# jcbowden/EagleEverything

Measured on NVIDIA B200. Metric: markers/s, higher is better.
Workload: dtype f64

## Files before the change

### eagleeverything_b200/csrc/capi.cu

```cuda
#include <cublas_v2.h>
#include <dlfcn.h>
#include <fcntl.h>
#include <sys/mman.h>
#include <sys/stat.h>
#include <unistd.h>

#include <cmath>
#include <cstdarg>
#include <cstdlib>
#include <cstring>
#include <atomic>
#include <condition_variable>
#include <functional>
#include <mutex>
#include <thread>
#include <unordered_map>
#include <string>
#include <vector>

#include "common.cuh"
#include "hostio.cuh"

struct eg_store {
    int8_t* d = nullptr;
// ... 74 lines not shown
    int dev = 0, sms = 0;
    if (cudaGetDevice(&dev) == cudaSuccess &&
        cudaDeviceGetAttribute(&sms, cudaDevAttrMultiProcessorCount, dev) == cudaSuccess && sms > 0)
        return sms;
    return 148;
}

static int ensure_init() {
    if (g_ctx.ready) return check_cuda(cudaSetDevice(g_ctx.device), "cudaSetDevice");
    const char* env = getenv("EAGLE_GPU_DEVICE");
    return eg_init(env ? atoi(env) : 0);
}

int ensure_init_pub() { return ensure_init(); }
cudaStream_t ctx_stream() { return g_ctx.stream; }
cublasHandle_t ctx_cublas() { return g_ctx.cublas; }

void syrk_release_cache();
void scan_i8_release();
void algebra_release();
void eigbasis_release();
void prep_i8_release();
int launch_prepare_i8(const double* d_S, const double* d_V, int64_t n, int64_t col0, int64_t col1, double* d_tmp,
                      double* d_Wp, int64_t Kpad, cudaStream_t st, bool* done);
static int g_scan_mode = -1;
int scan_mode() {
    if (g_scan_mode < 0) {
        const char* e = getenv("EAGLE_SCAN_MODE");
        g_scan_mode = (e && (e[0] == 'f' || e[0] == 'd' || e[0] == '0')) ? 0 : 1;
    }
    return g_scan_mode;
}
int launch_scan(const int8_t* d_Mt, int64_t L, int64_t n, int64_t pitch, const double* d_Wp,
                const int64_t* d_zero_rows, int n_zero, double* d_a, double* d_vara, cudaStream_t st);

#define g_pool_mu g_ctx.pool_mu
#define g_free_blocks g_ctx.free_blocks
#define g_live_blocks g_ctx.live_blocks
#define g_free_bytes g_ctx.free_bytes
#define g_recycle_limit g_ctx.recycle_limit

static void pool_flush_locked() {
    for (auto& b : g_free_blocks) cudaFreeAsync(b.p, g_ctx.stream);
    g_free_blocks.clear();
    g_free_bytes = 0;
}
static cudaError_t pool_alloc(void** p, size_t bytes) {
// ... 425 lines not shown
    cache_insert(key, s);
    *out = s;
    return EG_OK;
}

__global__ void __launch_bounds__(256) i8_to_f64_colmajor_kernel(const int8_t* __restrict__ in, int64_t rows,
                                                                 int64_t cols, int64_t pitch,
                                                                 double* __restrict__ out) {
    __shared__ int8_t tile[32][33];
    const int tx = threadIdx.x & 31, ty = threadIdx.x >> 5;
    const int64_t r0 = (int64_t)blockIdx.y * 32, c0 = (int64_t)blockIdx.x * 32;
    for (int i = ty; i < 32; i += 8) {
        const int64_t r = r0 + i, c = c0 + tx;
        tile[i][tx] = (r < rows && c < cols) ? in[r * pitch + c] : (int8_t)0;
    }
    __syncthreads();
    for (int i = ty; i < 32; i += 8) {
        const int64_t c = c0 + i, r = r0 + tx;
        if (r < rows && c < cols) out[r + c * rows] = -(double)tile[tx][i];
    }
}

__global__ void __launch_bounds__(256) symmetrize_upper_kernel(double* __restrict__ Wp, int64_t n, int64_t ld,
                                                               int w_is_upper) {
    __shared__ double tile[32][33];
    const int bx = blockIdx.x, by = blockIdx.y;
    if (bx < by) return;
    const int tx = threadIdx.x & 31, ty = threadIdx.x >> 5;
    const int64_t r0 = (int64_t)by * 32, c0 = (int64_t)bx * 32;
    for (int i = ty; i < 32; i += 8) {
        const int64_t r = c0 + tx, c = r0 + i;
        tile[i][tx] = (r < n && c < n) ? Wp[r + c * ld] : 0.0;
    }
    __syncthreads();
    for (int i = ty; i < 32; i += 8) {
        const int64_t r = r0 + tx, c = c0 + i;
        if (r < n && c < n) {
            if (r < c) Wp[r + c * ld] = Wp[r + c * ld] + (w_is_upper ? Wp[r + c * ld] : tile[tx][i]);
            else if (r > c) Wp[r + c * ld] = 0.0;
        }
    }
    if (bx != by) {
        __syncthreads();
        for (int i = ty; i < 32; i += 8) {
            const int64_t r = c0 + tx, c = r0 + i;
            if (r < n && c < n) Wp[r + c * ld] = 0.0;
        }
// ... 23 lines not shown
        const int64_t r = r0 + tx, c = c0 + i;
        v[k] = (r < n && c < n) ? A[r + c * n] : 0.0;
    }
    double mabs = 0.0, masym = 0.0;
#pragma unroll
    for (int k = 0; k < 16; k++) {
        const int i = ty + 4 * k;
        if (r0 + tx < n && c0 + i < n) {
            const double a = v[k], b = tile[tx][i];
            mabs = fmax(mabs, fmax(fabs(a), fabs(b)));
            const double d = fabs(a - b);
            masym = fmax(masym, d == d ? d : 1.0e300);
        }
    }
#pragma unroll
    for (int o = 16; o > 0; o >>= 1) {
        mabs = fmax(mabs, __shfl_xor_sync(0xffffffffu, mabs, o));
        masym = fmax(masym, __shfl_xor_sync(0xffffffffu, masym, o));
    }
    if ((threadIdx.x & 31) == 0) {
        atomicMax(out, (unsigned long long)__double_as_longlong(mabs));
        atomicMax(out + 1, (unsigned long long)__double_as_longlong(masym));
    }
}

static int partial_product(const eg_store* M, const std::vector<int64_t>& zero_cols, DevBuf& C, bool keep_product);
static int mmt_of_composite(const eg_store* M, const std::vector<int64_t>& zero_cols, double* out_host, bool keep_product);
static int scan_of_composite(const eg_store* Mt, const std::vector<int64_t>& zero_rows, const double* S, const double* V,
                             const double* a, double* out_a, double* out_vara);
static int mmt_of_store(const eg_store* M, const std::vector<int64_t>& zero_cols, double* out_host, bool keep_product = false) {
    Pin pin(M);
    if (M->nparts > 1) return mmt_of_composite(M, zero_cols, out_host, keep_product);
    const int64_t n = M->rows;
    DevBuf C, D;
    EG_TRY(partial_product(M, zero_cols, C, keep_product));
    EG_TRY(D.alloc((size_t)n * n * sizeof(double), "MMt output"));
    cudaStream_t st = g_ctx.stream;
    {
        Timer t(st);
        EG_TRY(eg_dev_mmt_finalize(C.as<int32_t>(), n, n, D.as<double>(), st));
        g_ctx.timing[2] = t.stop();
    }
    {
        Timer t(st);
        EG_TRY(d2h_staged(out_host, D.p, (size_t)n * n * sizeof(double), st));
        g_ctx.timing[3] = t.stop();
// ... 913 lines not shown
    const int64_t Kpad = round_up(n, 32), nc = col1 - col0;
    const bool want_i8 = eg_prep_uses_i8(n) != 0;
    if (upper_only && want_i8) {
        bool done = false;
        EG_TRY(launch_prepare_i8(d_S, d_V, n, col0, col1, d_tmp, d_Wp, Kpad, st, &done));
        if (done) return EG_OK;
    }
    const double one = 1.0, zero = 0.0;
    if (cublasSetStream(g_ctx.cublas, st) != CUBLAS_STATUS_SUCCESS) return set_error(EG_ERR_CUDA, "cublasSetStream");
    if (cublasDgemm(g_ctx.cublas, CUBLAS_OP_N, CUBLAS_OP_N, (int)n, (int)nc, (int)n, &one, d_V, (int)n, d_S + col0 * n,
                    (int)n, &zero, d_tmp, (int)n) != CUBLAS_STATUS_SUCCESS)
        return set_error(EG_ERR_CUDA, "cublasDgemm(V*S) failed");
    const int64_t step = upper_only ? 1024 : nc;
    for (int64_t b0 = 0; b0 < nc; b0 += step) {
        const int64_t nb = (b0 + step <= nc) ? step : nc - b0;
        const int64_t rows = upper_only ? (col0 + b0 + nb) : n;
        if (cublasDgemm(g_ctx.cublas, CUBLAS_OP_N, CUBLAS_OP_N, (int)rows, (int)nb, (int)n, &one, d_S, (int)n,
                        d_tmp + b0 * n, (int)n, &zero, d_Wp + (col0 + b0) * Kpad, (int)Kpad) != CUBLAS_STATUS_SUCCESS)
            return set_error(EG_ERR_CUDA, "cublasDgemm(S*tmp) failed");
    }
    return EG_OK;
}

extern "C" int eg_dev_scan_fold(const double* d_S, const double* d_a, int64_t n, int w_is_upper, double* d_Wp,
                                void* stream) {
    if (!d_S || !d_a || !d_Wp || n <= 0) return set_error(EG_ERR_ARG, "eg_dev_scan_fold: bad argument");
    EG_TRY(ensure_init());
    cudaStream_t st = (cudaStream_t)stream;
    const int64_t Kpad = round_up(n, 32);
    const double one = 1.0, zero = 0.0;
    if (cublasSetStream(g_ctx.cublas, st) != CUBLAS_STATUS_SUCCESS) return set_error(EG_ERR_CUDA, "cublasSetStream");
    if (cublasDgemv(g_ctx.cublas, CUBLAS_OP_N, (int)n, (int)n, &one, d_S, (int)n, d_a, 1, &zero, d_Wp + n * Kpad, 1) !=
        CUBLAS_STATUS_SUCCESS)
        return set_error(EG_ERR_CUDA, "cublasDgemv(S*a) failed");
    const unsigned nb = (unsigned)((n + 31) / 32);
    symmetrize_upper_kernel<<<dim3(nb, nb), 256, 0, st>>>(d_Wp, n, Kpad, w_is_upper);
    return check_launch("symmetrize_upper_kernel");
}

extern "C" int eg_dev_inputs_symmetric(const double* d_S, const double* d_V, int64_t n, int* yes, void* stream) {
    if (!yes) return set_error(EG_ERR_ARG, "null");
    double aS, dS, aV, dV;
    EG_TRY(eg_dev_symmetry(d_S, n, &aS, &dS, stream));
    EG_TRY(eg_dev_symmetry(d_V, n, &aV, &dV, stream));
    const char* env = getenv("EAGLE_SCAN_SYMMETRIC");
    *yes = !(env && env[0] == '0') && dS <= 1e-13 * aS && dV <= 1e-13 * aV;
    return EG_OK;
}

extern "C" int eg_dev_scan_prepare(const double* d_S, const double* d_V, const double* d_a, int64_t n, double* d_tmp,
                                   double* d_Wp, void* stream) {
    if (!d_S || !d_V || !d_a || !d_tmp || !d_Wp || n <= 0) return set_error(EG_ERR_ARG, "eg_dev_scan_prepare: bad argument");
    EG_TRY(ensure_init());
    int sym = 0;
    EG_TRY(eg_dev_inputs_symmetric(d_S, d_V, n, &sym, stream));
    EG_CUDA(cudaMemsetAsync(d_Wp, 0, (size_t)eg_scan_wp_elems(n) * 8, (cudaStream_t)stream));
    EG_TRY(eg_dev_scan_prepare_cols(d_S, d_V, n, 0, n, sym, d_tmp, d_Wp, stream));
    return eg_dev_scan_fold(d_S, d_a, n, sym, d_Wp, stream);
}

extern "C" int eg_ReadBlock(const char* asciifname, int64_t start_row, int64_t numcols, int64_t numrows_in_block,
                            double* out_colmajor) {
    if (!asciifname || !out_colmajor || start_row < 0 || numcols <= 0 || numrows_in_block <= 0)
        return set_error(EG_ERR_ARG, "ReadBlock: bad argument");
    EG_TRY(ensure_init());
    MappedFile f;
    EG_TRY(f.open_ro(asciifname));
    const void* nl = memchr(f.p, '\n', f.size);
    const int64_t line = nl ? (const uint8_t*)nl - f.p : (int64_t)f.size;
    if (numcols > line) return set_error(EG_ERR_FORMAT, "ReadBlock: lines of %s have %lld characters, %lld requested",
                                         asciifname, (long long)line, (long long)numcols);
    const int64_t nrows_file = ((int64_t)f.size + 1) / (line + 1);
    if (start_row + numrows_in_block > nrows_file)
        return set_error(EG_ERR_FORMAT, "ReadBlock: %s has %lld lines, rows [%lld,%lld) requested", asciifname,
                         (long long)nrows_file, (long long)start_row, (long long)(start_row + numrows_in_block));
    eg_store* s = nullptr;
// ... 651 lines not shown
```

### eagleeverything_b200/csrc/prep_i8.cu

```cuda
#include <cstdlib>
#include <vector>

#include "common.cuh"
#include "ptx.cuh"

namespace eg {

constexpr int PI_BM = 128;
constexpr int PI_BN = 256;
constexpr int PI_BK = 128;
constexpr int PI_STAGES = 4;
constexpr int PI_A_BYTES = PI_BM * PI_BK;
constexpr int PI_B_BYTES = PI_BN * PI_BK;
constexpr int PI_STAGE_BYTES = PI_A_BYTES + PI_B_BYTES;
constexpr int PI_THREADS = 192;
constexpr int PI_TMEM_COLS = 512;
constexpr int PI_SLICES = 7;
constexpr int PI_LEVELS = 7;
constexpr int PI_TERMS = PI_LEVELS * (PI_LEVELS + 1) / 2;
constexpr int PI_SMEM_BYTES = PI_STAGES * PI_STAGE_BYTES + 1024 + 256;
constexpr int PI_SROWS = 12;
constexpr int PI_PHASE = 8;
constexpr int PI_LAG = 4;

struct PrepParams {
    int64_t M, N, ld;
    double* out;
    const double* sL;
    const double* sR;
    int32_t lrow0, rrow0;
    int32_t KB;
    int64_t diag_shift;
    int32_t upper_only;
    const int2* tiles;
    int32_t ntiles, nchunks, ngroups;
    uint8_t tp[PI_TERMS], tq[PI_TERMS];
    uint8_t cbeg[PI_TERMS + 1];
    double cw[PI_TERMS];
    uint32_t* phase_ctr;
    int32_t phases_per_tile, phase_len, lag;
};

__device__ __forceinline__ void pi_red_add(uint32_t* p, uint32_t v) {
    asm volatile("red.relaxed.gpu.global.add.u32 [%0], %1;" ::"l"(p), "r"(v) : "memory");
}
__device__ __forceinline__ uint32_t pi_ld(const uint32_t* p) {
    uint32_t v;
    asm volatile("ld.relaxed.gpu.global.u32 %0, [%1];" : "=r"(v) : "l"(p) : "memory");
    return v;
}

__global__ void __launch_bounds__(PI_THREADS, 1)
prep_i8_kernel(const __grid_constant__ CUtensorMap tmapL, const __grid_constant__ CUtensorMap tmapR, const PrepParams p) {
    extern __shared__ uint8_t smem_raw[];
    uint8_t* smem = reinterpret_cast<uint8_t*>((reinterpret_cast<uintptr_t>(smem_raw) + 1023) & ~(uintptr_t)1023);
    uint64_t* bars = reinterpret_cast<uint64_t*>(smem + PI_STAGES * PI_STAGE_BYTES);
    uint64_t* full = bars;
    uint64_t* empty = bars + PI_STAGES;
    uint64_t* tmem_full = bars + 2 * PI_STAGES;
    uint64_t* tmem_empty = tmem_full + 2;
    uint32_t* tmem_slot = reinterpret_cast<uint32_t*>(tmem_empty + 2);

    const int warp = threadIdx.x >> 5, lane = threadIdx.x & 31;
    if (warp == 0 && lane == 0) {
        ptx::prefetch_tmap(&tmapL);
        ptx::prefetch_tmap(&tmapR);
        for (int s = 0; s < PI_STAGES; s++) {
            ptx::mbar_init(&full[s], 1);
            ptx::mbar_init(&empty[s], 1);
        }
        for (int a = 0; a < 2; a++) {
            ptx::mbar_init(&tmem_full[a], 1);
            ptx::mbar_init(&tmem_empty[a], 4);
        }
        ptx::fence_mbar_init();
    }
    if (warp == 1) ptx::tmem_alloc<PI_TMEM_COLS>(tmem_slot);
    ptx::tc_fence_before();
    __syncthreads();
    ptx::tc_fence_after();
    const uint32_t tmem_base = *tmem_slot;

    const int nun = p.ngroups * p.nchunks;

    if (warp == 0) {
// ... 85 lines not shown
                if (++acc == 2) { acc = 0; acc_phase ^= 1; }
            }
        }
    } else {
        const int q = warp & 3;
        int acc = 0;
        uint32_t acc_phase = 0;
        for (int u = 0; u < nun; u++) {
            const int gi = u / p.nchunks, c = u - gi * p.nchunks;
            const int tile = gi * (int)gridDim.x + (int)blockIdx.x;
            if (tile >= p.ntiles) break;
            const int2 t = p.tiles[tile];
            const bool first = c == 0, last = c == p.nchunks - 1;
            const double w = p.cw[c];
            const int64_t row0 = (int64_t)t.x * PI_BM + q * 32;
            const int64_t row = row0 + lane;
            const double srow = (last && row < p.M) ? p.sL[row] * 281474976710656.0  : 0.0;
            ptx::mbar_wait(&tmem_full[acc], acc_phase);
            ptx::tc_fence_after();
#pragma unroll 1
            for (int cc = 0; cc < PI_BN / 32; cc++) {
                const int64_t col0 = (int64_t)t.y * PI_BN + cc * 32;
                if (col0 >= p.N) continue;
                if (p.upper_only && col0 + 31 + p.diag_shift < row0) continue;
                uint32_t v[32];
                ptx::tmem_ld_32x32(tmem_base + ((uint32_t)(q * 32) << 16) + (uint32_t)(acc * PI_BN + cc * 32), v);
                double* o = p.out + row + col0 * p.ld;
                const bool live = row < p.M;
                double run[32];
#pragma unroll
                for (int j = 0; j < 32; j++) run[j] = (live && !first && col0 + j < p.N) ? o[(int64_t)j * p.ld] : 0.0;
                ptx::tmem_ld_wait();
                if (live) {
#pragma unroll
                    for (int j = 0; j < 32; j++) {
                        if (col0 + j < p.N) {
                            double x = w * (double)(int)v[j];
                            if (!first) x += run[j];
                            if (last) x *= srow * __ldg(p.sR + col0 + j);
                            o[(int64_t)j * p.ld] = x;
                        }
                    }
                }
            }
            ptx::tc_fence_before();
            __syncwarp();
            if (lane == 0) ptx::mbar_arrive(&tmem_empty[acc]);
// ... 6 lines not shown
    if (warp == 1) {
        ptx::tc_fence_after();
        ptx::tmem_dealloc<PI_TMEM_COLS>(tmem_base);
    }
}

constexpr int PP_STAGES = 6;
constexpr int PP_B_BYTES = 128 * PI_BK;
constexpr int PP_STAGE_BYTES = PI_A_BYTES + PP_B_BYTES;
constexpr int PP_SMEM_BYTES = PP_STAGES * PP_STAGE_BYTES + 1024 + 256;
constexpr int PP_BM = 2 * PI_BM;

__global__ void __launch_bounds__(PI_THREADS, 1)
prep_i8_pair_kernel(const __grid_constant__ CUtensorMap tmapL, const __grid_constant__ CUtensorMap tmapR, const PrepParams p) {
    extern __shared__ uint8_t smem_raw[];
    uint8_t* smem = reinterpret_cast<uint8_t*>((reinterpret_cast<uintptr_t>(smem_raw) + 1023) & ~(uintptr_t)1023);
    uint64_t* bars = reinterpret_cast<uint64_t*>(smem + PP_STAGES * PP_STAGE_BYTES);
    uint64_t* full = bars;
    uint64_t* empty = bars + PP_STAGES;
    uint64_t* tmem_full = bars + 2 * PP_STAGES;
    uint64_t* tmem_empty = tmem_full + 2;
    uint32_t* tmem_slot = reinterpret_cast<uint32_t*>(tmem_empty + 2);

    const int warp = threadIdx.x >> 5, lane = threadIdx.x & 31;
    const uint32_t rank = ptx::cluster_ctarank();
    const int cid = (int)ptx::cluster_id_x();
    const int ncl = (int)gridDim.x / 2;
    if (warp == 0 && lane == 0) {
        ptx::prefetch_tmap(&tmapL);
        ptx::prefetch_tmap(&tmapR);
        for (int s = 0; s < PP_STAGES; s++) {
            ptx::mbar_init(&full[s], 1);
            ptx::mbar_init(&empty[s], 1);
        }
        for (int a = 0; a < 2; a++) {
            ptx::mbar_init(&tmem_full[a], 1);
            ptx::mbar_init(&tmem_empty[a], 8);
        }
        ptx::fence_mbar_init();
    }
    if (warp == 1) ptx::tmem_alloc_pair<PI_TMEM_COLS>(tmem_slot);
    ptx::tc_fence_before();
    ptx::cluster_sync();
    ptx::tc_fence_after();
    const uint32_t tmem_base = *tmem_slot;

// ... 88 lines not shown
                if (++acc == 2) { acc = 0; acc_phase ^= 1; }
            }
        }
    } else {
        const int q = warp & 3;
        int acc = 0;
        uint32_t acc_phase = 0;
        for (int u = 0; u < nun; u++) {
            const int gi = u / p.nchunks, c = u - gi * p.nchunks;
            const int tile = gi * ncl + cid;
            if (tile >= p.ntiles) break;
            const int2 t = p.tiles[tile];
            const bool first = c == 0, last = c == p.nchunks - 1;
            const double w = p.cw[c];
            const int64_t row0 = (int64_t)t.x * PP_BM + (int64_t)rank * PI_BM + q * 32;
            const int64_t row = row0 + lane;
            const double srow = (last && row < p.M) ? p.sL[row] * 281474976710656.0  : 0.0;
            ptx::mbar_wait(&tmem_full[acc], acc_phase);
            ptx::tc_fence_after();
#pragma unroll 1
            for (int cc = 0; cc < PI_BN / 32; cc++) {
                const int64_t col0 = (int64_t)t.y * PI_BN + cc * 32;
                if (col0 >= p.N) continue;
                if (p.upper_only && col0 + 31 + p.diag_shift < row0) continue;
                uint32_t v[32];
                ptx::tmem_ld_32x32(tmem_base + ((uint32_t)(q * 32) << 16) + (uint32_t)(acc * PI_BN + cc * 32), v);
                double* o = p.out + row + col0 * p.ld;
                const bool live = row < p.M;
                double run[32];
#pragma unroll
                for (int j = 0; j < 32; j++) run[j] = (live && !first && col0 + j < p.N) ? o[(int64_t)j * p.ld] : 0.0;
                ptx::tmem_ld_wait();
                if (live) {
#pragma unroll
                    for (int j = 0; j < 32; j++) {
                        if (col0 + j < p.N) {
                            double x = w * (double)(int)v[j];
                            if (!first) x += run[j];
                            if (last) x *= srow * __ldg(p.sR + col0 + j);
                            o[(int64_t)j * p.ld] = x;
                        }
                    }
                }
            }
            ptx::tc_fence_before();
            __syncwarp();
            if (lane == 0) ptx::mbar_arrive_cluster(ptx::mapa(ptx::smem_u32(&tmem_empty[acc]), 0));
            if (++acc == 2) { acc = 0; acc_phase ^= 1; }
        }
    }

    ptx::tc_fence_before();
    ptx::cluster_sync();
    if (warp == 1) {
        ptx::tc_fence_after();
        ptx::tmem_dealloc_pair<PI_TMEM_COLS>(tmem_base);
    }
}

__global__ void __launch_bounds__(256) pi_colscale_kernel(const double* __restrict__ A, int64_t rows, int64_t ld,
                                                          int32_t* __restrict__ expo, double* __restrict__ scale,
                                                          const double* __restrict__ rowscale) {
    const int64_t c = blockIdx.x;
    unsigned long long m = 0;
    for (int64_t i = threadIdx.x; i < rows; i += 256) {
        const double x = rowscale ? A[i + c * ld] * rowscale[i] : A[i + c * ld];
        const unsigned long long b = (unsigned long long)__double_as_longlong(x) & 0x7FFFFFFFFFFFFFFFull;
        m = b > m ? b : m;
    }
    __shared__ unsigned long long sh[8];
#pragma unroll
    for (int o = 16; o > 0; o >>= 1) {
        const unsigned long long other = __shfl_xor_sync(0xffffffffu, m, o);
        m = other > m ? other : m;
    }
    if ((threadIdx.x & 31) == 0) sh[threadIdx.x >> 5] = m;
    __syncthreads();
    if (threadIdx.x == 0) {
        for (int w = 1; w < 8; w++) m = sh[w] > m ? sh[w] : m;
        const double amax = __longlong_as_double((long long)m);
        int e = 0;
        double s = 0.0;
        if (m >= 0x7FF0000000000000ull) {
            s = __longlong_as_double(0x7FF8000000000000LL);
        } else if (amax > 0.0) {
            if (frexp(amax, &e) >= 0.9921875) e++;
            s = ldexp(1.0, e - 55);
        }
        expo[c] = e;
        scale[c] = s;
    }
}
__global__ void __launch_bounds__(256) pi_slice_kernel(const double* __restrict__ A, int64_t rows, int64_t ld,
                                                       const int32_t* __restrict__ expo, int8_t* __restrict__ Q, int64_t Kp,
                                                       int64_t slice_stride, const double* __restrict__ rowscale) {
    const int64_t c = blockIdx.y;
    const int64_t i0 = ((int64_t)blockIdx.x * 256 + threadIdx.x) * 4;
    if (i0 >= Kp) return;
    uint32_t out[PI_SLICES];
#pragma unroll
    for (int s = 0; s < PI_SLICES; s++) out[s] = 0;
    const int e = expo[c];
#pragma unroll
    for (int d = 0; d < 4; d++) {
        const int64_t i = i0 + d;
        if (i < rows) {
            const double xs = ldexp(rowscale ? A[i + c * ld] * rowscale[i] : A[i + c * ld], 55 - e);
            long long X = fabs(xs) < 3.6e16 ? __double2ll_rn(xs) : 0;
#pragma unroll
            for (int s = PI_SLICES - 1; s > 0; s--) {
                const int q = (int)(int8_t)(X & 0xFF);
                out[s] |= ((uint32_t)q & 0xFFu) << (8 * d);
                X = (X - q) >> 8;
            }
            out[0] |= ((uint32_t)(int)X & 0xFFu) << (8 * d);
        }
    }
    int8_t* base = Q + c * Kp + i0;
#pragma unroll
    for (int s = 0; s < PI_SLICES; s++) *reinterpret_cast<uint32_t*>(base + (int64_t)s * slice_stride) = out[s];
}

typedef CUresult (*PFN_encodeTiled)(CUtensorMap*, CUtensorMapDataType, cuuint32_t, void*, const cuuint64_t*,
                                    const cuuint64_t*, const cuuint32_t*, const cuuint32_t*, CUtensorMapInterleave,
                                    CUtensorMapSwizzle, CUtensorMapL2promotion, CUtensorMapFloatOOBfill);
static PFN_encodeTiled pi_encode_fn() {
    static PFN_encodeTiled fn = nullptr;
    if (!fn) {
        void* f = nullptr;
        cudaDriverEntryPointQueryResult qres;
        if (cudaGetDriverEntryPoint("cuTensorMapEncodeTiled", &f, cudaEnableDefault, &qres) == cudaSuccess &&
            qres == cudaDriverEntryPointSuccess)
            fn = reinterpret_cast<PFN_encodeTiled>(f);
    }
    return fn;
}
static int pi_make_map(CUtensorMap* m, const void* base, int64_t Kp, int64_t rows) {
    PFN_encodeTiled enc = pi_encode_fn();
    if (!enc) return set_error(EG_ERR_CUDA, "cuTensorMapEncodeTiled is not available");
    const cuuint64_t gdim[3] = {(cuuint64_t)Kp, (cuuint64_t)rows, (cuuint64_t)PI_SLICES};
    const cuuint64_t gstride[2] = {(cuuint64_t)Kp, (cuuint64_t)(Kp * rows)};
    const cuuint32_t box[3] = {128, 128, 1};
    const cuuint32_t estr[3] = {1, 1, 1};
    CUresult r = enc(m, CU_TENSOR_MAP_DATA_TYPE_UINT8, 3, const_cast<void*>(base), gdim, gstride, box, estr,
                     CU_TENSOR_MAP_INTERLEAVE_NONE, CU_TENSOR_MAP_SWIZZLE_128B, CU_TENSOR_MAP_L2_PROMOTION_L2_256B,
                     CU_TENSOR_MAP_FLOAT_OOB_FILL_NONE);
    if (r != CUDA_SUCCESS) return set_error(EG_ERR_CUDA, "cuTensorMapEncodeTiled failed (%d)", (int)r);
    return EG_OK;
}

static bool prep_i8_pair() {
    const char* e = getenv("EAGLE_PREP_PAIR");
    return e && e[0] == '1';
}

struct PrepWorkspace {
    int device = -1;
    int8_t* qS = nullptr;  size_t qS_cap = 0;
    int8_t* qV = nullptr;  size_t qV_cap = 0;
    int8_t* qX = nullptr;  size_t qX_cap = 0;
    double* sc = nullptr;  size_t sc_cap = 0;
    int32_t* ex = nullptr; size_t ex_cap = 0;
    int2* tiles = nullptr; size_t tiles_cap = 0;
    uint32_t* phase = nullptr; size_t phase_cap = 0;
};
static thread_local PrepWorkspace g_pi;

static thread_local cudaEvent_t g_pi_ev[4] = {nullptr, nullptr, nullptr, nullptr};
static thread_local double g_pi_ops = 0.0;
static thread_local int g_pi_marks = 0;
void prep_kernel_times(double* ms, double* ops) {
    *ms = 0.0;
    *ops = g_pi_ops;
    for (int i = 0; i + 1 < g_pi_marks; i += 2) {
        float f = 0.f;
        if (cudaEventSynchronize(g_pi_ev[i + 1]) == cudaSuccess && cudaEventElapsedTime(&f, g_pi_ev[i], g_pi_ev[i + 1]) == cudaSuccess)
            *ms += f;
    }
}

void prep_i8_release() {
    cudaFree(g_pi.qS); cudaFree(g_pi.qV); cudaFree(g_pi.qX); cudaFree(g_pi.sc); cudaFree(g_pi.ex); cudaFree(g_pi.tiles); cudaFree(g_pi.phase);
    g_pi = PrepWorkspace();
}
template <class T>
static bool pi_grow(T** ptr, size_t* cap, size_t need) {
    if (need <= *cap && *ptr) return true;
    if (*ptr) cudaFree(*ptr);
    *ptr = nullptr;
    *cap = 0;
    if (malloc_retry((void**)ptr, need * sizeof(T)) != cudaSuccess) {
        cudaGetLastError();
        return false;
    }
    *cap = need;
    return true;
}

static int pi_slice(const double* d_A, int64_t rows, int64_t ld, int64_t ncols, int8_t* Q, int64_t Kp, int32_t* expo,
                    double* scale, cudaStream_t st, const double* d_rowscale = nullptr) {
    pi_colscale_kernel<<<(unsigned)ncols, 256, 0, st>>>(d_A, rows, ld, expo, scale, d_rowscale);
    EG_TRY(check_launch("pi_colscale_kernel"));
    pi_slice_kernel<<<dim3((unsigned)((Kp / 4 + 255) / 256), (unsigned)ncols), 256, 0, st>>>(d_A, rows, ld, expo, Q, Kp,
                                                                                          Kp * ncols, d_rowscale);
    return check_launch("pi_slice_kernel");
}

static int pi_product(const int8_t* qL, int64_t lrows, const double* sL, int64_t lrow0, int64_t M, const int8_t* qR,
                      int64_t rrows, const double* sR, int64_t rrow0, int64_t N, int64_t n, int64_t Kp, double* out,
                      int64_t ld, bool upper_only, int64_t diag_shift, cudaStream_t st) {
    const bool pair = prep_i8_pair();
    const int BMt = pair ? PP_BM : PI_BM;
    const int TM = (int)((M + BMt - 1) / BMt), TN = (int)((N + PI_BN - 1) / PI_BN);
    std::vector<int2> h;
    int srows = PI_SROWS;
    if (const char* e = getenv("EAGLE_PREP_SROWS")) srows = atoi(e) > 0 ? atoi(e) : srows;
    if (pair) srows = (srows + 1) / 2;
    for (int sr = 0; sr < TM; sr += srows)
        for (int tj = 0; tj < TN; tj++)
            for (int ti = sr; ti < TM && ti < sr + srows; ti++) {
                if (upper_only && (int64_t)(tj + 1) * PI_BN - 1 + diag_shift < (int64_t)ti * BMt) continue;
                h.push_back(make_int2(ti, tj));
            }
    if (h.empty()) return EG_OK;
    if (!pi_grow(&g_pi.tiles, &g_pi.tiles_cap, h.size())) return set_error(EG_ERR_ALLOC, "prep_i8: tile table");
    EG_CUDA(cudaMemcpyAsync(g_pi.tiles, h.data(), h.size() * sizeof(int2), cudaMemcpyHostToDevice, st));
    EG_CUDA(cudaStreamSynchronize(st));

    PrepParams p;
    p.M = M; p.N = N; p.ld = ld; p.out = out;
    p.sL = sL + lrow0; p.sR = sR + rrow0;
    p.lrow0 = (int32_t)lrow0; p.rrow0 = (int32_t)rrow0;
    p.KB = (int32_t)(Kp / PI_BK);
    p.diag_shift = diag_shift;
    p.upper_only = upper_only ? 1 : 0;
    p.tiles = g_pi.tiles;
    p.ntiles = (int32_t)h.size();
    const int64_t tmax64 = (((int64_t)1 << 31) - 1) / (n * 16384);
    const int tmax = (int)(tmax64 > PI_LEVELS ? PI_LEVELS : tmax64);
    if (tmax < 1) return set_error(EG_ERR_ARG, "prep_i8: n = %lld too large for int32 accumulation", (long long)n);
    int nt = 0, nc = 0;
    for (int d = PI_LEVELS - 1; d >= 0; d--) {
        for (int p0 = 0; p0 <= d; p0 += tmax) {
            p.cbeg[nc] = (uint8_t)nt;
            double w = 1.0;
            for (int e = 0; e < PI_LEVELS - 1 - d; e++) w *= 256.0;
            p.cw[nc] = w;
            for (int pp = p0; pp <= d && pp < p0 + tmax; pp++) {
                p.tp[nt] = (uint8_t)pp;
                p.tq[nt] = (uint8_t)(d - pp);
                nt++;
            }
            nc++;
        }
    }
    p.cbeg[nc] = (uint8_t)nt;
    p.nchunks = nc;
    const int sms = num_sms();
    const int workers_max = pair ? sms / 2 : sms;
    const int workers = p.ntiles < workers_max ? p.ntiles : workers_max;
    const int grid = pair ? 2 * workers : workers;
    p.ngroups = (p.ntiles + workers - 1) / workers;

    CUtensorMap tL, tR;
    EG_TRY(pi_make_map(&tL, qL, Kp, lrows));
    EG_TRY(pi_make_map(&tR, qR, Kp, rrows));
    if (pair) EG_CUDA(cudaFuncSetAttribute(prep_i8_pair_kernel, cudaFuncAttributeMaxDynamicSharedMemorySize, PP_SMEM_BYTES));
    else EG_CUDA(cudaFuncSetAttribute(prep_i8_kernel, cudaFuncAttributeMaxDynamicSharedMemorySize, PI_SMEM_BYTES));
    p.phase_len = PI_PHASE;
    p.lag = PI_LAG;
    if (const char* e = getenv("EAGLE_PREP_PHASE")) p.phase_len = atoi(e) > 0 ? atoi(e) : p.phase_len;
    if (const char* e = getenv("EAGLE_PREP_LAG")) p.lag = atoi(e) > 0 && atoi(e) <= 8 ? atoi(e) : p.lag;
    p.phases_per_tile = (nt * p.KB + p.phase_len - 1) / p.phase_len;
    const size_t nctr = (size_t)p.ngroups * p.phases_per_tile;
    const char* env_fc = getenv("EAGLE_PREP_FLOWCTL");
    const bool flow = !(env_fc && env_fc[0] == '0') && workers > 1;
    p.phase_ctr = nullptr;
    if (flow) {
        if (!pi_grow(&g_pi.phase, &g_pi.phase_cap, nctr)) return set_error(EG_ERR_ALLOC, "prep_i8: flow-control counters");
        EG_CUDA(cudaMemsetAsync(g_pi.phase, 0, nctr * sizeof(uint32_t), st));
        p.phase_ctr = g_pi.phase;
    }
    cudaLaunchConfig_t cfg = {};
    cfg.gridDim = dim3((unsigned)grid);
    cfg.blockDim = dim3(PI_THREADS);
    cfg.dynamicSmemBytes = pair ? PP_SMEM_BYTES : PI_SMEM_BYTES;
    cfg.stream = st;
    cudaLaunchAttribute attr[2];
    attr[0].id = cudaLaunchAttributeCooperative;
    attr[0].val.cooperative = flow ? 1 : 0;
    attr[1].id = cudaLaunchAttributeClusterDimension;
    attr[1].val.clusterDim.x = 2;
    attr[1].val.clusterDim.y = 1;
    attr[1].val.clusterDim.z = 1;
    cfg.attrs = attr;
    cfg.numAttrs = pair ? 2 : 1;
    if (!g_pi_ev[0])
        for (int i = 0; i < 4; i++) cudaEventCreate(&g_pi_ev[i]);
    if (g_pi_marks <= 2) {
        cudaEventRecord(g_pi_ev[g_pi_marks], st);
        g_pi_ops += (double)p.ntiles * nt * p.KB * 2.0 * BMt * PI_BN * PI_BK;
    }
    if (pair) EG_CUDA(cudaLaunchKernelEx(&cfg, prep_i8_pair_kernel, tL, tR, p));
    else EG_CUDA(cudaLaunchKernelEx(&cfg, prep_i8_kernel, tL, tR, p));
    if (g_pi_marks <= 2) {
        cudaEventRecord(g_pi_ev[g_pi_marks + 1], st);
        g_pi_marks += 2;
    }
    return check_launch("prep_i8_kernel");
}

int launch_prepare_i8(const double* d_S, const double* d_V, int64_t n, int64_t col0, int64_t col1, double* d_tmp,
                      double* d_Wp, int64_t Kpad, cudaStream_t st, bool* done) {
    *done = false;
    g_pi_marks = 0;
    g_pi_ops = 0.0;
    int dev = 0;
    EG_CUDA(cudaGetDevice(&dev));
    if (g_pi.device != dev) {
        if (g_pi.device >= 0) prep_i8_release();
        g_pi.device = dev;
    }
    if (n * 16384 >= ((int64_t)1 << 31)) return EG_OK;
    const int64_t Kp = round_up(n, 128), nc = col1 - col0;
    size_t free_b = 0, total_b = 0;
    EG_CUDA(cudaMemGetInfo(&free_b, &total_b));
    const size_t need = (size_t)PI_SLICES * Kp * (size_t)(2 * n + nc);
    const size_t have = g_pi.qS_cap + g_pi.qV_cap + g_pi.qX_cap;
    if (need > have && need - have + ((size_t)2 << 30) > free_b) return EG_OK;
    if (!pi_grow(&g_pi.qS, &g_pi.qS_cap, (size_t)PI_SLICES * Kp * n) || !pi_grow(&g_pi.qV, &g_pi.qV_cap, (size_t)PI_SLICES * Kp * n) ||
        !pi_grow(&g_pi.qX, &g_pi.qX_cap, (size_t)PI_SLICES * Kp * nc) || !pi_grow(&g_pi.sc, &g_pi.sc_cap, (size_t)(2 * n + nc)) ||
        !pi_grow(&g_pi.ex, &g_pi.ex_cap, (size_t)(2 * n + nc)))
        return EG_OK;
    double *sS = g_pi.sc, *sV = g_pi.sc + n, *sX = g_pi.sc + 2 * n;
    int32_t *eS = g_pi.ex, *eV = g_pi.ex + n, *eX = g_pi.ex + 2 * n;
    EG_TRY(pi_slice(d_S, n, n, n, g_pi.qS, Kp, eS, sS, st));
    EG_TRY(pi_slice(d_V, n, n, n, g_pi.qV, Kp, eV, sV, st));
    EG_TRY(pi_product(g_pi.qV, n, sV, 0, n, g_pi.qS, n, sS, col0, nc, n, Kp, d_tmp, n, false, 0, st));
    EG_TRY(pi_slice(d_tmp, n, n, nc, g_pi.qX, Kp, eX, sX, st));
    EG_TRY(pi_product(g_pi.qS, n, sS, 0, col1, g_pi.qX, nc, sX, 0, nc, n, Kp, d_Wp + col0 * Kpad, Kpad, true, col0, st));
    *done = true;
    return EG_OK;
}

int launch_prepare_eig_i8(const double* d_Ut, const double* d_rs, int64_t n, double* d_Wp, int64_t Kpad, cudaStream_t st,
                          bool* done) {
    *done = false;
    g_pi_marks = 0;
    g_pi_ops = 0.0;
    int dev = 0;
    EG_CUDA(cudaGetDevice(&dev));
    if (g_pi.device != dev) {
        if (g_pi.device >= 0) prep_i8_release();
        g_pi.device = dev;
    }
    if (n * 16384 >= ((int64_t)1 << 31)) return EG_OK;
    const int64_t Kp = round_up(n, 128);
    size_t free_b = 0, total_b = 0;
    EG_CUDA(cudaMemGetInfo(&free_b, &total_b));
    const size_t need = (size_t)PI_SLICES * Kp * (size_t)n;
    if (need > g_pi.qS_cap && need - g_pi.qS_cap + ((size_t)2 << 30) > free_b) return EG_OK;
    if (!pi_grow(&g_pi.qS, &g_pi.qS_cap, need) || !pi_grow(&g_pi.sc, &g_pi.sc_cap, (size_t)n) ||
        !pi_grow(&g_pi.ex, &g_pi.ex_cap, (size_t)n))
        return EG_OK;
    EG_TRY(pi_slice(d_Ut, n, n, n, g_pi.qS, Kp, g_pi.ex, g_pi.sc, st, d_rs));
    EG_TRY(pi_product(g_pi.qS, n, g_pi.sc, 0, n, g_pi.qS, n, g_pi.sc, 0, n, n, Kp, d_Wp, Kpad, true, 0, st));
    *done = true;
    return EG_OK;
}

}
```

Baseline: 2.949 million.

## Decide scan-prepare symmetry on device and cache tile tables to remove host syncs

The symmetry check for S and V now stays on the GPU: a device flag is computed and then read by the slice, transpose, product and symmetrize kernels, so the host no longer waits on the result. Asymmetric inputs are handled by device-gated transposes and an extra lower-triangle product launch that exits early when the inputs are symmetric. Per-shape tile tables are cached on the device instead of being uploaded with a stream synchronize on every product, and shared-memory attributes and memory-info queries are done only once. The cost is extra launches that do nothing (transposes, lower pass) in the symmetric case, plus more complex control flow.

```diff
diff --git a/eagleeverything_b200/csrc/capi.cu b/eagleeverything_b200/csrc/capi.cu
--- a/eagleeverything_b200/csrc/capi.cu
+++ b/eagleeverything_b200/csrc/capi.cu
@@ -120,7 +120,8 @@
 void eigbasis_release();
 void prep_i8_release();
 int launch_prepare_i8(const double* d_S, const double* d_V, int64_t n, int64_t col0, int64_t col1, double* d_tmp,
-                      double* d_Wp, int64_t Kpad, cudaStream_t st, bool* done);
+                      double* d_Wp, int64_t Kpad, cudaStream_t st, bool* done, const int* d_sym = nullptr);
+int prep_i8_reserve(int64_t n, int64_t nc, bool* ok);
 static int g_scan_mode = -1;
 int scan_mode() {
     if (g_scan_mode < 0) {
@@ -592,7 +593,8 @@
 }
 
 __global__ void __launch_bounds__(256) symmetrize_upper_kernel(double* __restrict__ Wp, int64_t n, int64_t ld,
-                                                               int w_is_upper) {
+                                                               int w_is_upper, const int* __restrict__ d_w_is_upper) {
+    if (d_w_is_upper) w_is_upper = *d_w_is_upper;
     __shared__ double tile[32][33];
     const int bx = blockIdx.x, by = blockIdx.y;
     if (bx < by) return;
@@ -662,6 +664,12 @@
         atomicMax(out, (unsigned long long)__double_as_longlong(mabs));
         atomicMax(out + 1, (unsigned long long)__double_as_longlong(masym));
     }
+}
+
+__global__ void inputs_symmetric_kernel(const unsigned long long* __restrict__ m, int allow, int* __restrict__ flag) {
+    const double aS = __longlong_as_double((long long)m[0]), dS = __longlong_as_double((long long)m[1]);
+    const double aV = __longlong_as_double((long long)m[2]), dV = __longlong_as_double((long long)m[3]);
+    *flag = allow && dS <= 1e-13 * aS && dV <= 1e-13 * aV;
 }
 
 static int partial_product(const eg_store* M, const std::vector<int64_t>& zero_cols, DevBuf& C, bool keep_product);
@@ -1621,11 +1629,8 @@
     return EG_OK;
 }
 
-extern "C" int eg_dev_scan_fold(const double* d_S, const double* d_a, int64_t n, int w_is_upper, double* d_Wp,
-                                void* stream) {
-    if (!d_S || !d_a || !d_Wp || n <= 0) return set_error(EG_ERR_ARG, "eg_dev_scan_fold: bad argument");
-    EG_TRY(ensure_init());
-    cudaStream_t st = (cudaStream_t)stream;
+static int scan_fold(const double* d_S, const double* d_a, int64_t n, int w_is_upper, const int* d_w_is_upper,
+                     double* d_Wp, cudaStream_t st) {
     const int64_t Kpad = round_up(n, 32);
     const double one = 1.0, zero = 0.0;
     if (cublasSetStream(g_ctx.cublas, st) != CUBLAS_STATUS_SUCCESS) return set_error(EG_ERR_CUDA, "cublasSetStream");
@@ -1633,8 +1638,14 @@
         CUBLAS_STATUS_SUCCESS)
         return set_error(EG_ERR_CUDA, "cublasDgemv(S*a) failed");
     const unsigned nb = (unsigned)((n + 31) / 32);
-    symmetrize_upper_kernel<<<dim3(nb, nb), 256, 0, st>>>(d_Wp, n, Kpad, w_is_upper);
+    symmetrize_upper_kernel<<<dim3(nb, nb), 256, 0, st>>>(d_Wp, n, Kpad, w_is_upper, d_w_is_upper);
     return check_launch("symmetrize_upper_kernel");
+}
+extern "C" int eg_dev_scan_fold(const double* d_S, const double* d_a, int64_t n, int w_is_upper, double* d_Wp,
+                                void* stream) {
+    if (!d_S || !d_a || !d_Wp || n <= 0) return set_error(EG_ERR_ARG, "eg_dev_scan_fold: bad argument");
+    EG_TRY(ensure_init());
+    return scan_fold(d_S, d_a, n, w_is_upper, nullptr, d_Wp, (cudaStream_t)stream);
 }
 
 extern "C" int eg_dev_inputs_symmetric(const double* d_S, const double* d_V, int64_t n, int* yes, void* stream) {
@@ -1647,10 +1658,43 @@
     return EG_OK;
 }
 
+static int inputs_symmetric_dev(const double* d_S, const double* d_V, int64_t n, cudaStream_t st, const int** d_flag) {
+    static thread_local unsigned long long* work[64] = {};
+    int dev = 0;
+    EG_CUDA(cudaGetDevice(&dev));
+    if (dev < 0 || dev >= 64) return set_error(EG_ERR_ARG, "device %d", dev);
+    unsigned long long*& w = work[dev];
+    if (!w) EG_CUDA(cudaMalloc(&w, 5 * sizeof(unsigned long long)));
+    EG_CUDA(cudaMemsetAsync(w, 0, 4 * sizeof(unsigned long long), st));
+    const unsigned nb = (unsigned)((n + 63) / 64);
+    symmetry_kernel<<<dim3(nb, nb), 256, 0, st>>>(d_S, n, w);
+    EG_TRY(check_launch("symmetry_kernel"));
+    symmetry_kernel<<<dim3(nb, nb), 256, 0, st>>>(d_V, n, w + 2);
+    EG_TRY(check_launch("symmetry_kernel"));
+    const char* env = getenv("EAGLE_SCAN_SYMMETRIC");
+    int* flag = reinterpret_cast<int*>(w + 4);
+    inputs_symmetric_kernel<<<1, 1, 0, st>>>(w, !(env && env[0] == '0'), flag);
+    EG_TRY(check_launch("inputs_symmetric_kernel"));
+    *d_flag = flag;
+    return EG_OK;
+}
+
 extern "C" int eg_dev_scan_prepare(const double* d_S, const double* d_V, const double* d_a, int64_t n, double* d_tmp,
                                    double* d_Wp, void* stream) {
     if (!d_S || !d_V || !d_a || !d_tmp || !d_Wp || n <= 0) return set_error(EG_ERR_ARG, "eg_dev_scan_prepare: bad argument");
     EG_TRY(ensure_init());
+    cudaStream_t st = (cudaStream_t)stream;
+    bool fits = false;
+    if (eg_prep_uses_i8(n)) EG_TRY(prep_i8_reserve(n, n, &fits));
+    if (fits) {
+        const int* d_sym = nullptr;
+        EG_TRY(inputs_symmetric_dev(d_S, d_V, n, st, &d_sym));
+        EG_CUDA(cudaMemsetAsync(d_Wp, 0, (size_t)eg_scan_wp_elems(n) * 8, st));
+        bool done = false;
+        EG_TRY(launch_prepare_i8(d_S, d_V, n, 0, n, d_tmp, d_Wp, round_up(n, 32), st, &done, d_sym));
+        if (!done) return set_error(EG_ERR_ALLOC, "eg_dev_scan_prepare: digit-slice workspace lost");
+        return scan_fold(d_S, d_a, n, 0, d_sym, d_Wp, st);
+    }
     int sym = 0;
     EG_TRY(eg_dev_inputs_symmetric(d_S, d_V, n, &sym, stream));
     EG_CUDA(cudaMemsetAsync(d_Wp, 0, (size_t)eg_scan_wp_elems(n) * 8, (cudaStream_t)stream));
diff --git a/eagleeverything_b200/csrc/prep_i8.cu b/eagleeverything_b200/csrc/prep_i8.cu
--- a/eagleeverything_b200/csrc/prep_i8.cu
+++ b/eagleeverything_b200/csrc/prep_i8.cu
@@ -39,6 +39,8 @@
     double cw[PI_TERMS];
     uint32_t* phase_ctr;
     int32_t phases_per_tile, phase_len, lag;
+    const int* sym;
+    int32_t exit_if_sym;
 };
 
 __device__ __forceinline__ void pi_red_add(uint32_t* p, uint32_t v) {
@@ -61,6 +63,9 @@
     uint64_t* tmem_empty = tmem_full + 2;
     uint32_t* tmem_slot = reinterpret_cast<uint32_t*>(tmem_empty + 2);
 
+    const bool asym = p.sym && *p.sym == 0;
+    if (p.exit_if_sym && !asym) return;
+    const bool upper_only = p.upper_only && !asym;
     const int warp = threadIdx.x >> 5, lane = threadIdx.x & 31;
     if (warp == 0 && lane == 0) {
         ptx::prefetch_tmap(&tmapL);
@@ -192,7 +197,7 @@
             for (int cc = 0; cc < PI_BN / 32; cc++) {
                 const int64_t col0 = (int64_t)t.y * PI_BN + cc * 32;
                 if (col0 >= p.N) continue;
-                if (p.upper_only && col0 + 31 + p.diag_shift < row0) continue;
+                if (upper_only && col0 + 31 + p.diag_shift < row0) continue;
                 uint32_t v[32];
                 ptx::tmem_ld_32x32(tmem_base + ((uint32_t)(q * 32) << 16) + (uint32_t)(acc * PI_BN + cc * 32), v);
                 double* o = p.out + row + col0 * p.ld;
@@ -245,6 +250,9 @@
     uint64_t* tmem_empty = tmem_full + 2;
     uint32_t* tmem_slot = reinterpret_cast<uint32_t*>(tmem_empty + 2);
 
+    const bool asym = p.sym && *p.sym == 0;
+    if (p.exit_if_sym && !asym) return;
+    const bool upper_only = p.upper_only && !asym;
     const int warp = threadIdx.x >> 5, lane = threadIdx.x & 31;
     const uint32_t rank = ptx::cluster_ctarank();
     const int cid = (int)ptx::cluster_id_x();
@@ -379,7 +387,7 @@
             for (int cc = 0; cc < PI_BN / 32; cc++) {
                 const int64_t col0 = (int64_t)t.y * PI_BN + cc * 32;
                 if (col0 >= p.N) continue;
-                if (p.upper_only && col0 + 31 + p.diag_shift < row0) continue;
+                if (upper_only && col0 + 31 + p.diag_shift < row0) continue;
                 uint32_t v[32];
                 ptx::tmem_ld_32x32(tmem_base + ((uint32_t)(q * 32) << 16) + (uint32_t)(acc * PI_BN + cc * 32), v);
                 double* o = p.out + row + col0 * p.ld;
@@ -415,9 +423,15 @@
     }
 }
 
-__global__ void __launch_bounds__(256) pi_colscale_kernel(const double* __restrict__ A, int64_t rows, int64_t ld,
+__device__ __forceinline__ const double* pi_source(const double* A, const double* At, const int* sym) {
+    return (sym && *sym == 0) ? At : A;
+}
+__global__ void __launch_bounds__(256) pi_colscale_kernel(const double* __restrict__ A_, int64_t rows, int64_t ld,
                                                           int32_t* __restrict__ expo, double* __restrict__ scale,
-                                                          const double* __restrict__ rowscale) {
+                                                          const double* __restrict__ rowscale, const double* At,
+                                                          const int* sym) {
+    const double* __restrict__ A = pi_source(A_, At, sym);
+    if (!A) return;
     const int64_t c = blockIdx.x;
     unsigned long long m = 0;
     for (int64_t i = threadIdx.x; i < rows; i += 256) {
@@ -448,9 +462,12 @@
         scale[c] = s;
     }
 }
-__global__ void __launch_bounds__(256) pi_slice_kernel(const double* __restrict__ A, int64_t rows, int64_t ld,
+__global__ void __launch_bounds__(256) pi_slice_kernel(const double* __restrict__ A_, int64_t rows, int64_t ld,
                                                        const int32_t* __restrict__ expo, int8_t* __restrict__ Q, int64_t Kp,
-                                                       int64_t slice_stride, const double* __restrict__ rowscale) {
+                                                       int64_t slice_stride, const double* __restrict__ rowscale,
+                                                       const double* At, const int* sym) {
+    const double* __restrict__ A = pi_source(A_, At, sym);
+    if (!A) return;
     const int64_t c = blockIdx.y;
     const int64_t i0 = ((int64_t)blockIdx.x * 256 + threadIdx.x) * 4;
     if (i0 >= Kp) return;
@@ -476,6 +493,27 @@
     int8_t* base = Q + c * Kp + i0;
 #pragma unroll
     for (int s = 0; s < PI_SLICES; s++) *reinterpret_cast<uint32_t*>(base + (int64_t)s * slice_stride) = out[s];
+}
+
+__global__ void __launch_bounds__(256) pi_transpose_kernel(const double* __restrict__ A, int64_t n, double* __restrict__ At,
+                                                           const int* __restrict__ sym) {
+    if (*sym) return;
+    __shared__ double tile[32][33];
+    const int tx = threadIdx.x & 31, ty = threadIdx.x >> 5;
+    const int64_t nt = (n + 31) / 32;
+    for (int64_t t = blockIdx.x; t < nt * nt; t += gridDim.x) {
+        const int64_t r0 = (t % nt) * 32, c0 = (t / nt) * 32;
+        for (int i = ty; i < 32; i += 8) {
+            const int64_t r = r0 + tx, c = c0 + i;
+            tile[i][tx] = (r < n && c < n) ? A[r + c * n] : 0.0;
+        }
+        __syncthreads();
+        for (int i = ty; i < 32; i += 8) {
+            const int64_t r = c0 + tx, c = r0 + i;
+            if (r < n && c < n) At[r + c * n] = tile[tx][i];
+        }
+        __syncthreads();
+    }
 }
 
 typedef CUresult (*PFN_encodeTiled)(CUtensorMap*, CUtensorMapDataType, cuuint32_t, void*, const cuuint64_t*,
@@ -518,10 +556,23 @@
     int8_t* qX = nullptr;  size_t qX_cap = 0;
     double* sc = nullptr;  size_t sc_cap = 0;
     int32_t* ex = nullptr; size_t ex_cap = 0;
-    int2* tiles = nullptr; size_t tiles_cap = 0;
     uint32_t* phase = nullptr; size_t phase_cap = 0;
+    bool smem_attrs = false;
 };
 static thread_local PrepWorkspace g_pi;
+
+enum { PI_ALL = 0, PI_UPPER = 1, PI_LOWER = 2 };
+struct TileTable {
+    int64_t M, N, diag_shift;
+    int bm, srows, part;
+    int2* d;
+    int count;
+};
+static thread_local std::vector<TileTable> g_pi_tiles;
+static void pi_tiles_release() {
+    for (auto& t : g_pi_tiles) cudaFree(t.d);
+    g_pi_tiles.clear();
+}
 
 static thread_local cudaEvent_t g_pi_ev[4] = {nullptr, nullptr, nullptr, nullptr};
 static thread_local double g_pi_ops = 0.0;
@@ -537,7 +588,8 @@
 }
 
 void prep_i8_release() {
-    cudaFree(g_pi.qS); cudaFree(g_pi.qV); cudaFree(g_pi.qX); cudaFree(g_pi.sc); cudaFree(g_pi.ex); cudaFree(g_pi.tiles); cudaFree(g_pi.phase);
+    cudaFree(g_pi.qS); cudaFree(g_pi.qV); cudaFree(g_pi.qX); cudaFree(g_pi.sc); cudaFree(g_pi.ex); cudaFree(g_pi.phase);
+    pi_tiles_release();
     g_pi = PrepWorkspace();
 }
 template <class T>
@@ -555,34 +607,68 @@
 }
 
 static int pi_slice(const double* d_A, int64_t rows, int64_t ld, int64_t ncols, int8_t* Q, int64_t Kp, int32_t* expo,
-                    double* scale, cudaStream_t st, const double* d_rowscale = nullptr) {
-    pi_colscale_kernel<<<(unsigned)ncols, 256, 0, st>>>(d_A, rows, ld, expo, scale, d_rowscale);
+                    double* scale, cudaStream_t st, const double* d_rowscale = nullptr, const double* d_At = nullptr,
+                    const int* d_sym = nullptr) {
+    pi_colscale_kernel<<<(unsigned)ncols, 256, 0, st>>>(d_A, rows, ld, expo, scale, d_rowscale, d_At, d_sym);
     EG_TRY(check_launch("pi_colscale_kernel"));
     pi_slice_kernel<<<dim3((unsigned)((Kp / 4 + 255) / 256), (unsigned)ncols), 256, 0, st>>>(d_A, rows, ld, expo, Q, Kp,
-                                                                                          Kp * ncols, d_rowscale);
+                                                                                          Kp * ncols, d_rowscale, d_At, d_sym);
     return check_launch("pi_slice_kernel");
+}
+
+static int pi_transpose(const double* d_A, int64_t n, double* d_At, const int* d_sym, cudaStream_t st) {
+    pi_transpose_kernel<<<(unsigned)(num_sms() * 4), 256, 0, st>>>(d_A, n, d_At, d_sym);
+    return check_launch("pi_transpose_kernel");
+}
+
+static int pi_tile_table(int64_t M, int64_t N, int bm, int srows, int part, int64_t diag_shift, cudaStream_t st,
+                         const TileTable** out) {
+    for (const auto& t : g_pi_tiles)
+        if (t.M == M && t.N == N && t.bm == bm && t.srows == srows && t.part == part && t.diag_shift == diag_shift) {
+            *out = &t;
+            return EG_OK;
+        }
+    if (g_pi_tiles.size() >= 64) {
+        EG_CUDA(cudaStreamSynchronize(st));
+        pi_tiles_release();
+    }
+    const int TM = (int)((M + bm - 1) / bm), TN = (int)((N + PI_BN - 1) / PI_BN);
+    std::vector<int2> h;
+    for (int sr = 0; sr < TM; sr += srows)
+        for (int tj = 0; tj < TN; tj++)
+            for (int ti = sr; ti < TM && ti < sr + srows; ti++) {
+                const bool upper = (int64_t)(tj + 1) * PI_BN - 1 + diag_shift >= (int64_t)ti * bm;
+                if ((part == PI_UPPER && !upper) || (part == PI_LOWER && upper)) continue;
+                h.push_back(make_int2(ti, tj));
+            }
+    TileTable t{M, N, diag_shift, bm, srows, part, nullptr, (int)h.size()};
+    if (!h.empty()) {
+        if (malloc_retry((void**)&t.d, h.size() * sizeof(int2)) != cudaSuccess) {
+            cudaGetLastError();
+            return set_error(EG_ERR_ALLOC, "prep_i8: tile table");
+        }
+        const cudaError_t e = cudaMemcpy(t.d, h.data(), h.size() * sizeof(int2), cudaMemcpyHostToDevice);
+        if (e != cudaSuccess) {
+            cudaFree(t.d);
+            return check_cuda(e, "prep_i8: tile table upload");
+        }
+    }
+    g_pi_tiles.push_back(t);
+    *out = &g_pi_tiles.back();
+    return EG_OK;
 }
 
 static int pi_product(const int8_t* qL, int64_t lrows, const double* sL, int64_t lrow0, int64_t M, const int8_t* qR,
                       int64_t rrows, const double* sR, int64_t rrow0, int64_t N, int64_t n, int64_t Kp, double* out,
-                      int64_t ld, bool upper_only, int64_t diag_shift, cudaStream_t st) {
+                      int64_t ld, int part, int64_t diag_shift, cudaStream_t st, const int* d_sym = nullptr) {
     const bool pair = prep_i8_pair();
     const int BMt = pair ? PP_BM : PI_BM;
-    const int TM = (int)((M + BMt - 1) / BMt), TN = (int)((N + PI_BN - 1) / PI_BN);
-    std::vector<int2> h;
     int srows = PI_SROWS;
     if (const char* e = getenv("EAGLE_PREP_SROWS")) srows = atoi(e) > 0 ? atoi(e) : srows;
     if (pair) srows = (srows + 1) / 2;
-    for (int sr = 0; sr < TM; sr += srows)
-        for (int tj = 0; tj < TN; tj++)
-            for (int ti = sr; ti < TM && ti < sr + srows; ti++) {
-                if (upper_only && (int64_t)(tj + 1) * PI_BN - 1 + diag_shift < (int64_t)ti * BMt) continue;
-                h.push_back(make_int2(ti, tj));
-            }
-    if (h.empty()) return EG_OK;
-    if (!pi_grow(&g_pi.tiles, &g_pi.tiles_cap, h.size())) return set_error(EG_ERR_ALLOC, "prep_i8: tile table");
-    EG_CUDA(cudaMemcpyAsync(g_pi.tiles, h.data(), h.size() * sizeof(int2), cudaMemcpyHostToDevice, st));
-    EG_CUDA(cudaStreamSynchronize(st));
+    const TileTable* tt = nullptr;
+    EG_TRY(pi_tile_table(M, N, BMt, srows, part, diag_shift, st, &tt));
+    if (tt->count == 0) return EG_OK;
 
     PrepParams p;
     p.M = M; p.N = N; p.ld = ld; p.out = out;
@@ -590,9 +676,11 @@
     p.lrow0 = (int32_t)lrow0; p.rrow0 = (int32_t)rrow0;
     p.KB = (int32_t)(Kp / PI_BK);
     p.diag_shift = diag_shift;
-    p.upper_only = upper_only ? 1 : 0;
-    p.tiles = g_pi.tiles;
-    p.ntiles = (int32_t)h.size();
+    p.upper_only = part == PI_UPPER ? 1 : 0;
+    p.sym = d_sym;
+    p.exit_if_sym = part == PI_LOWER ? 1 : 0;
+    p.tiles = tt->d;
+    p.ntiles = tt->count;
     const int64_t tmax64 = (((int64_t)1 << 31) - 1) / (n * 16384);
     const int tmax = (int)(tmax64 > PI_LEVELS ? PI_LEVELS : tmax64);
     if (tmax < 1) return set_error(EG_ERR_ARG, "prep_i8: n = %lld too large for int32 accumulation", (long long)n);
@@ -622,8 +710,11 @@
     CUtensorMap tL, tR;
     EG_TRY(pi_make_map(&tL, qL, Kp, lrows));
     EG_TRY(pi_make_map(&tR, qR, Kp, rrows));
-    if (pair) EG_CUDA(cudaFuncSetAttribute(prep_i8_pair_kernel, cudaFuncAttributeMaxDynamicSharedMemorySize, PP_SMEM_BYTES));
-    else EG_CUDA(cudaFuncSetAttribute(prep_i8_kernel, cudaFuncAttributeMaxDynamicSharedMemorySize, PI_SMEM_BYTES));
+    if (!g_pi.smem_attrs) {
+        EG_CUDA(cudaFuncSetAttribute(prep_i8_pair_kernel, cudaFuncAttributeMaxDynamicSharedMemorySize, PP_SMEM_BYTES));
+        EG_CUDA(cudaFuncSetAttribute(prep_i8_kernel, cudaFuncAttributeMaxDynamicSharedMemorySize, PI_SMEM_BYTES));
+        g_pi.smem_attrs = true;
+    }
     p.phase_len = PI_PHASE;
     p.lag = PI_LAG;
     if (const char* e = getenv("EAGLE_PREP_PHASE")) p.phase_len = atoi(e) > 0 ? atoi(e) : p.phase_len;
@@ -667,35 +758,59 @@
     return check_launch("prep_i8_kernel");
 }
 
+static void pi_use_device() {
+    int dev = 0;
+    if (cudaGetDevice(&dev) != cudaSuccess) return;
+    if (g_pi.device != dev) {
+        if (g_pi.device >= 0) prep_i8_release();
+        g_pi.device = dev;
+    }
+}
+
+int prep_i8_reserve(int64_t n, int64_t nc, bool* ok) {
+    *ok = false;
+    pi_use_device();
+    if (n * 16384 >= ((int64_t)1 << 31)) return EG_OK;
+    const int64_t Kp = round_up(n, 128);
+    const size_t qn = (size_t)PI_SLICES * Kp * n, qx = (size_t)PI_SLICES * Kp * nc;
+    if (qn > g_pi.qS_cap || qn > g_pi.qV_cap || qx > g_pi.qX_cap) {
+        size_t free_b = 0, total_b = 0;
+        EG_CUDA(cudaMemGetInfo(&free_b, &total_b));
+        const size_t need = 2 * qn + qx;
+        const size_t have = g_pi.qS_cap + g_pi.qV_cap + g_pi.qX_cap;
+        if (need > have && need - have + ((size_t)2 << 30) > free_b) return EG_OK;
+    }
+    *ok = pi_grow(&g_pi.qS, &g_pi.qS_cap, qn) && pi_grow(&g_pi.qV, &g_pi.qV_cap, qn) && pi_grow(&g_pi.qX, &g_pi.qX_cap, qx) &&
+          pi_grow(&g_pi.sc, &g_pi.sc_cap, (size_t)(2 * n + nc)) && pi_grow(&g_pi.ex, &g_pi.ex_cap, (size_t)(2 * n + nc));
+    return EG_OK;
+}
+
 int launch_prepare_i8(const double* d_S, const double* d_V, int64_t n, int64_t col0, int64_t col1, double* d_tmp,
-                      double* d_Wp, int64_t Kpad, cudaStream_t st, bool* done) {
+                      double* d_Wp, int64_t Kpad, cudaStream_t st, bool* done, const int* d_sym) {
     *done = false;
     g_pi_marks = 0;
     g_pi_ops = 0.0;
-    int dev = 0;
-    EG_CUDA(cudaGetDevice(&dev));
-    if (g_pi.device != dev) {
-        if (g_pi.device >= 0) prep_i8_release();
-        g_pi.device = dev;
-    }
-    if (n * 16384 >= ((int64_t)1 << 31)) return EG_OK;
+    if (d_sym && (col0 != 0 || col1 != n)) return set_error(EG_ERR_ARG, "prep_i8: a device-decided product needs all columns");
     const int64_t Kp = round_up(n, 128), nc = col1 - col0;
-    size_t free_b = 0, total_b = 0;
-    EG_CUDA(cudaMemGetInfo(&free_b, &total_b));
-    const size_t need = (size_t)PI_SLICES * Kp * (size_t)(2 * n + nc);
-    const size_t have = g_pi.qS_cap + g_pi.qV_cap + g_pi.qX_cap;
-    if (need > have && need - have + ((size_t)2 << 30) > free_b) return EG_OK;
-    if (!pi_grow(&g_pi.qS, &g_pi.qS_cap, (size_t)PI_SLICES * Kp * n) || !pi_grow(&g_pi.qV, &g_pi.qV_cap, (size_t)PI_SLICES * Kp * n) ||
-        !pi_grow(&g_pi.qX, &g_pi.qX_cap, (size_t)PI_SLICES * Kp * nc) || !pi_grow(&g_pi.sc, &g_pi.sc_cap, (size_t)(2 * n + nc)) ||
-        !pi_grow(&g_pi.ex, &g_pi.ex_cap, (size_t)(2 * n + nc)))
-        return EG_OK;
+    bool ok = false;
+    EG_TRY(prep_i8_reserve(n, nc, &ok));
+    if (!ok) return EG_OK;
     double *sS = g_pi.sc, *sV = g_pi.sc + n, *sX = g_pi.sc + 2 * n;
     int32_t *eS = g_pi.ex, *eV = g_pi.ex + n, *eX = g_pi.ex + 2 * n;
     EG_TRY(pi_slice(d_S, n, n, n, g_pi.qS, Kp, eS, sS, st));
-    EG_TRY(pi_slice(d_V, n, n, n, g_pi.qV, Kp, eV, sV, st));
-    EG_TRY(pi_product(g_pi.qV, n, sV, 0, n, g_pi.qS, n, sS, col0, nc, n, Kp, d_tmp, n, false, 0, st));
+    if (d_sym) EG_TRY(pi_transpose(d_V, n, d_tmp, d_sym, st));
+    EG_TRY(pi_slice(d_V, n, n, n, g_pi.qV, Kp, eV, sV, st, nullptr, d_tmp, d_sym));
+    EG_TRY(pi_product(g_pi.qV, n, sV, 0, n, g_pi.qS, n, sS, col0, nc, n, Kp, d_tmp, n, PI_ALL, 0, st));
     EG_TRY(pi_slice(d_tmp, n, n, nc, g_pi.qX, Kp, eX, sX, st));
-    EG_TRY(pi_product(g_pi.qS, n, sS, 0, col1, g_pi.qX, nc, sX, 0, nc, n, Kp, d_Wp + col0 * Kpad, Kpad, true, col0, st));
+    if (d_sym) {
+        EG_TRY(pi_transpose(d_S, n, d_tmp, d_sym, st));
+        EG_TRY(pi_slice(nullptr, n, n, n, g_pi.qS, Kp, eS, sS, st, nullptr, d_tmp, d_sym));
+    }
+    EG_TRY(pi_product(g_pi.qS, n, sS, 0, col1, g_pi.qX, nc, sX, 0, nc, n, Kp, d_Wp + col0 * Kpad, Kpad, PI_UPPER, col0, st,
+                      d_sym));
+    if (d_sym)
+        EG_TRY(pi_product(g_pi.qS, n, sS, 0, col1, g_pi.qX, nc, sX, 0, nc, n, Kp, d_Wp + col0 * Kpad, Kpad, PI_LOWER, col0,
+                          st, d_sym));
     *done = true;
     return EG_OK;
 }
@@ -705,23 +820,20 @@
     *done = false;
     g_pi_marks = 0;
     g_pi_ops = 0.0;
-    int dev = 0;
-    EG_CUDA(cudaGetDevice(&dev));
-    if (g_pi.device != dev) {
-        if (g_pi.device >= 0) prep_i8_release();
-        g_pi.device = dev;
-    }
+    pi_use_device();
     if (n * 16384 >= ((int64_t)1 << 31)) return EG_OK;
     const int64_t Kp = round_up(n, 128);
-    size_t free_b = 0, total_b = 0;
-    EG_CUDA(cudaMemGetInfo(&free_b, &total_b));
     const size_t need = (size_t)PI_SLICES * Kp * (size_t)n;
-    if (need > g_pi.qS_cap && need - g_pi.qS_cap + ((size_t)2 << 30) > free_b) return EG_OK;
+    if (need > g_pi.qS_cap) {
+        size_t free_b = 0, total_b = 0;
+        EG_CUDA(cudaMemGetInfo(&free_b, &total_b));
+        if (need - g_pi.qS_cap + ((size_t)2 << 30) > free_b) return EG_OK;
+    }
     if (!pi_grow(&g_pi.qS, &g_pi.qS_cap, need) || !pi_grow(&g_pi.sc, &g_pi.sc_cap, (size_t)n) ||
         !pi_grow(&g_pi.ex, &g_pi.ex_cap, (size_t)n))
         return EG_OK;
     EG_TRY(pi_slice(d_Ut, n, n, n, g_pi.qS, Kp, g_pi.ex, g_pi.sc, st, d_rs));
-    EG_TRY(pi_product(g_pi.qS, n, g_pi.sc, 0, n, g_pi.qS, n, g_pi.sc, 0, n, n, Kp, d_Wp, Kpad, true, 0, st));
+    EG_TRY(pi_product(g_pi.qS, n, g_pi.sc, 0, n, g_pi.qS, n, g_pi.sc, 0, n, n, Kp, d_Wp, Kpad, PI_UPPER, 0, st));
     *done = true;
     return EG_OK;
 }
```

Measured after the change: 2.970 million (median of 6 runs). No clear change (+0.7%).
